# swyoon/Diffusion-by-MaxEntIRL

Hardware: AMD Instinct MI355X
Metric: images/sec (CIFAR-10 DDPM T=10 generation) (higher is better)
Workload: dtype bf16; 1 GPU; CIFAR-10 DDPM U-Net (35.7M params) VARSampler T=10 generation, 256 images/GPU/step, 3x32x32 (BASELINE configs[1]); noise drawn inside the step; global_batch=256, T=10, parallelism=dp1 (independent trajectories, no collective)

## Files before the change

### diffusion-by-maxentirl_amd/csrc/conv1x1_rw.hip

```cpp
#include "conv_common.h"
#include "gn_common.h"

namespace {

#define RW_GPTR(p) ((const __attribute__((address_space(1))) void*)(p))
#define RW_LPTR(p) ((__attribute__((address_space(3))) void*)(p))
#define RW_WAIT_VM(n) asm volatile("s_waitcnt vmcnt(%0)" ::"n"(n) : "memory")
__device__ __forceinline__ void rw_barrier() { asm volatile("s_waitcnt lgkmcnt(0)\n\ts_barrier" ::: "memory"); }

constexpr int RW_CHUNK = 64 * 256;
constexpr int RW_RO = 64 * 256;
constexpr int RW_TBL = 128 * 8;

struct RwGn {
    const float* ab;
    bf16* y;
    int HW, silu;
};

__device__ __forceinline__ void rw_wait_vm(int n) {
    switch (__builtin_amdgcn_readfirstlane(n)) {
#define RW_C(k) case k: RW_WAIT_VM(k); break;
#define RW_C8(k) RW_C(k) RW_C(k + 1) RW_C(k + 2) RW_C(k + 3) RW_C(k + 4) RW_C(k + 5) RW_C(k + 6) RW_C(k + 7)
    RW_C8(0) RW_C8(8) RW_C8(16) RW_C8(24) RW_C8(32) RW_C8(40) RW_C8(48) RW_C8(56)
#undef RW_C8
#undef RW_C
    default: RW_WAIT_VM(0);
    }
}

template <int NCH, int R, bool RES, bool GN>
__global__ __launch_bounds__(256, ((NCH > 3 || R > 4) ? 1 : 2)) void conv1x1_rw_kernel(ConvArgs p, RwGn q) {
    static_assert(R - 1 <= 4 * NCH && R >= 3 && 4 * (R - 2) + 4 * (RES ? 8 : 4) < 64, "ring depth");
    static_assert(!(GN && RES) && (!GN || 5 * (R - 2) + 4 * 4 + 4 * (R - 1) < 64), "GN side output: no residual, vmcnt range");
    constexpr int BOPS = RES ? 8 : 4;
    constexpr int NYOUNG = 4 * (R - 2);
    extern __shared__ __attribute__((aligned(1024))) char smem[];
    char* const ring = smem;

    const int tid = threadIdx.x, lane = tid & 63, h = lane >> 5;
    const int wave = __builtin_amdgcn_readfirstlane(tid >> 6);
    char* const ro = smem + R * RW_CHUNK + wave * 4096;
    char* const tbl = smem + R * RW_CHUNK + RW_RO;
    const int xcd = blockIdx.x & 7, j = blockIdx.x >> 3;
    const int cot = j % p.CT;
    const int nstreams = (gridDim.x >> 3) / p.CT * 8;
    const int stream = (j / p.CT) * 8 + xcd;
    const int ntiles = stream < p.PT ? (p.PT - stream + nstreams - 1) / nstreams : 0;
    if (ntiles == 0) return;

    bf16x8 A[NCH * 8];
// ... 35 lines not shown
                                             RW_LPTR(ring + slot * RW_CHUNK + (wave * 4 + u) * 1024), 16, 0, 0);
    };
    int rpx[4], rc8[4];
#pragma unroll
    for (int i = 0; i < 4; ++i) {
        rpx[i] = i * 16 + (lane >> 2);
        rc8[i] = ((lane & 3) ^ ((rpx[i] >> 1) & 3)) * 8;
    }
    auto tile_off = [&](int tile, int i) -> size_t {
        return ((size_t)(stream + tile * nstreams) * 64 + rpx[i]) * p.Cout + cot * 128 + wave * 32 + rc8[i];
    };
    auto issue_residual = [&](int tile) {
#pragma unroll
        for (int i = 0; i < 4; ++i)
            __builtin_amdgcn_global_load_lds(RW_GPTR(p.residual + tile_off(tile, i)), RW_LPTR(ro + i * 1024), 16, 0, 0);
    };

    const int gtot = ntiles * NCH;
    if (RES) issue_residual(0);
#pragma unroll
    for (int g = 0; g < R - 1; ++g)
        if (g < gtot) issue_chunk(g / NCH, g % NCH, g);

    int boff[8];
    {
        const int px = lane & 31;
#pragma unroll
        for (int ks = 0; ks < 8; ++ks) boff[ks] = px * 256 + (((ks * 2 + h) ^ (px & 15)) << 4);
    }

    const int gnp = GN ? 4 / p.CT : 0;
    const int gs = tid & 15, gpx0 = cot * (64 / p.CT) + (tid >> 4);

    int slot = 0;
    for (int ti = 0; ti < ntiles; ++ti) {
        f32x16 acc[2];
#pragma unroll
        for (int nb = 0; nb < 2; ++nb)
#pragma unroll
            for (int r = 0; r < 16; ++r) acc[nb][r] = 0.f;
#pragma unroll
        for (int c = 0; c < NCH; ++c) {
            const int g = ti * NCH + c;
            const int kmax = R - 1 - c > 0 ? (R - 1 - c + NCH - 1) / NCH : 0;
            const int nbnd = ti < kmax ? ti : kmax;
            if (g + R - 2 >= gtot) RW_WAIT_VM(0);
            else if (GN) rw_wait_vm(5 * (R - 2) + nbnd * BOPS + (g < R - 1 ? g : R - 1) * gnp);
            else if (nbnd == 0) RW_WAIT_VM(NYOUNG);
            else if (nbnd == 1) RW_WAIT_VM(NYOUNG + BOPS);
            else if (nbnd == 2) RW_WAIT_VM(NYOUNG + 2 * BOPS);
            else if (nbnd == 3) RW_WAIT_VM(NYOUNG + 3 * BOPS);
            else RW_WAIT_VM(NYOUNG + 4 * BOPS);
            rw_barrier();
            {
                const int gi = g + R - 1;
                const int si = slot == 0 ? R - 1 : slot - 1;
                if (gi < gtot) issue_chunk(ti + (c + R - 1) / NCH, (c + R - 1) % NCH, si);
            }
            const char* img = ring + slot * RW_CHUNK;
#pragma unroll
            for (int ks = 0; ks < 8; ++ks)
#pragma unroll
                for (int nb = 0; nb < 2; ++nb) {
                    const bf16x8 b = *reinterpret_cast<const bf16x8*>(img + boff[ks] + nb * (32 * 256));
                    acc[nb] = __builtin_amdgcn_mfma_f32_32x32x16_bf16(A[c * 8 + ks], b, acc[nb], 0, 0, 0);
                }
            if constexpr (GN) {
                float ga[8], gb[8];
                const f32x4* t = reinterpret_cast<const f32x4*>(tbl + slot * RW_TBL + gs * 64);
#pragma unroll
                for (int i = 0; i < 4; ++i) {
                    const f32x4 v = t[i];
                    ga[2 * i] = v[0]; gb[2 * i] = v[1]; ga[2 * i + 1] = v[2]; gb[2 * i + 1] = v[3];
                }
                bf16* const yt = q.y + (size_t)(stream + ti * nstreams) * 64 * (NCH * 128) + c * 128 + gs * 8;
                for (int i = 0; i < gnp; ++i) {
                    const int px = gpx0 + 16 * i;
                    const bf16x8 v = *reinterpret_cast<const bf16x8*>(img + px * 256 + ((gs ^ (px & 15)) << 4));
                    *reinterpret_cast<bf16x8*>(yt + (size_t)px * (NCH * 128)) = gn_norm8(v, ga, gb, q.silu);
                }
            }
            slot = slot + 1 == R ? 0 : slot + 1;
        }
        if (RES) {
            if ((ti + 1) * NCH + R - 1 > gtot) RW_WAIT_VM(0);
            else RW_WAIT_VM(4 * NCH);
        }
#pragma unroll
        for (int nb = 0; nb < 2; ++nb) {
            const int px = nb * 32 + (lane & 31);
#pragma unroll
            for (int g4 = 0; g4 < 4; ++g4) {
                char* a = ro + px * 64 + ((g4 ^ ((px >> 1) & 3)) << 4) + 8 * h;
                f32x4 v;
#pragma unroll
                for (int e = 0; e < 4; ++e) v[e] = acc[nb][4 * g4 + e] + bv[g4][e];
                if (RES) {
                    const bf16x4 r = *reinterpret_cast<const bf16x4*>(a);
#pragma unroll
                    for (int e = 0; e < 4; ++e) v[e] += (float)r[e];
                }
                bf16x4 o;
#pragma unroll
                for (int e = 0; e < 4; ++e) o[e] = (bf16)dxmi_act_lin(v[e], slope);
                *reinterpret_cast<bf16x4*>(a) = o;
            }
        }
        asm volatile("s_waitcnt lgkmcnt(0)" ::: "memory");
        {
            bf16x8 v[4];
#pragma unroll
            for (int i = 0; i < 4; ++i) v[i] = *reinterpret_cast<const bf16x8*>(ro + i * 1024 + lane * 16);
#pragma unroll
            for (int i = 0; i < 4; ++i) *reinterpret_cast<bf16x8*>(reinterpret_cast<bf16*>(p.out) + tile_off(ti, i)) = v[i];
        }
        if (RES && ti + 1 < ntiles) issue_residual(ti + 1);
    }
}

template <int NCH, int R>
int rw_launch(const ConvPlan& p, hipStream_t st) {
    static bool attr_set = false;
    if (!attr_set) {
        (void)hipFuncSetAttribute(reinterpret_cast<const void*>(conv1x1_rw_kernel<NCH, R, true, false>), hipFuncAttributeMaxDynamicSharedMemorySize, 160 * 1024);
        (void)hipFuncSetAttribute(reinterpret_cast<const void*>(conv1x1_rw_kernel<NCH, R, false, false>), hipFuncAttributeMaxDynamicSharedMemorySize, 160 * 1024);
        attr_set = true;
    }
    const RwGn none = {};
    if (p.args.residual) hipLaunchKernelGGL((conv1x1_rw_kernel<NCH, R, true, false>), dim3(p.grid), dim3(256), p.lds, st, p.args, none);
    else hipLaunchKernelGGL((conv1x1_rw_kernel<NCH, R, false, false>), dim3(p.grid), dim3(256), p.lds, st, p.args, none);
    DXMI_CHECK_LAUNCH("dxmi_conv2d_fwd(1x1 rw)");
    return DXMI_OK;
}

template <int NCH, int R>
int rw_launch_gn(const ConvArgs& b, const RwGn& g, int grid, hipStream_t st) {
    const size_t lds = (size_t)R * (RW_CHUNK + RW_TBL) + RW_RO;
    static bool attr_set = false;
    if (!attr_set) {
        (void)hipFuncSetAttribute(reinterpret_cast<const void*>(conv1x1_rw_kernel<NCH, R, false, true>), hipFuncAttributeMaxDynamicSharedMemorySize, 160 * 1024);
        attr_set = true;
    }
    hipLaunchKernelGGL((conv1x1_rw_kernel<NCH, R, false, true>), dim3(grid), dim3(256), lds, st, b, g);
    DXMI_CHECK_LAUNCH("dxmi_groupnorm_silu_shortcut");
    return DXMI_OK;
}

int rw_grid(ConvArgs& b) {
    const int K = b.C0 + b.C1;
    b.PT = (int)((long)b.N * b.OH * b.OW / 64);
// ... 11 lines not shown
    const int K = a.C0 + a.C1;
    if (K % 128 != 0 || a.C0 % 128 != 0 || K > 512 || a.Cout % 128 != 0 || a.Cout / 128 > 32) return false;
    const long px = (long)a.N * a.OH * a.OW;
    if (px % 64 != 0 || px / 64 < 512) return false;
    const int nch = K / 128;
    p->kind = ConvKernel::rw; p->t0 = nch; p->t1 = nch > 3 ? 6 : 3;
    p->grid = rw_grid(p->args);
    p->lds = (size_t)p->t1 * RW_CHUNK + RW_RO;
    p->id = 500000 + nch * 1000 + p->t1 * 10 + (a.residual ? 1 : 0);
    return true;
}

int conv1x1_rw_launch(const ConvPlan& p, hipStream_t st) {
    switch (p.t0) {
    case 1: return rw_launch<1, 3>(p, st);
    case 2: return rw_launch<2, 3>(p, st);
    case 3: return rw_launch<3, 3>(p, st);
    default: return rw_launch<4, 6>(p, st);
    }
}

static int gn_shortcut_nch(const dxmi_conv_desc* d, int groups) {
    if (!d || d->ksize != 1 || d->stride != 1 || d->pad != 0 || d->upsample || d->residual || d->addvec || d->mask_src || d->gn_stats ||
        d->gn_out || d->act != DXMI_ACT_NONE || d->variant != 0 || d->in_mode != DXMI_IN_NHWC_BF16 || d->out_mode != DXMI_OUT_NHWC_BF16)
        return 0;
    const int K = d->C0 + d->C1, CT = d->Cout / 128;
    if (d->IH != d->OH || d->IW != d->OW || (d->OH * d->OW) % 64 != 0) return 0;
    if (CT != 1 && CT != 2 && CT != 4) return 0;
    if (groups <= 0 || groups > 32 || K % groups != 0 || (K / groups) % 2 != 0 || d->C1 % 8 != 0) return 0;
    ConvPlan p;
    return conv_plan(d, &p) == DXMI_OK && p.kind == ConvKernel::rw ? p.t0 : 0;
}

extern "C" int dxmi_groupnorm_silu_shortcut_supported(const dxmi_conv_desc* d, int32_t groups) {
    return gn_shortcut_nch(d, groups) > 0 ? 1 : 0;
}

extern "C" int dxmi_groupnorm_silu_shortcut(const dxmi_conv_desc* d, const float* stats0, int32_t P0, const float* stats1, int32_t P1,
                                            const float* gamma, const float* beta, int32_t groups, float eps, int32_t apply_silu, void* y,
                                            float* ab_workspace, void* stream) {
    DXMI_CHECK_ARG(d && d->in0 && d->wpacked && d->out && y && ab_workspace && stats0 && gamma && beta && P0 > 0,
                   "dxmi_groupnorm_silu_shortcut: null pointer");
    DXMI_CHECK_ARG(d->C1 == 0 || (d->in1 && stats1 && P1 > 0), "dxmi_groupnorm_silu_shortcut: C1>0 needs in1 and stats1");
    const int nch = gn_shortcut_nch(d, groups);
    if (nch == 0) return 1;
    const int HW = d->OH * d->OW;
    int rc = gn_finalize_launch(stats0, P0, d->C0, stats1, P1, d->C1, gamma, beta, ab_workspace, d->N, HW, groups, eps, (hipStream_t)stream);
    if (rc != DXMI_OK) return rc;
    ConvArgs b = {};
    b.in0 = (const bf16*)d->in0; b.in1 = (const bf16*)d->in1; b.w = (const bf16*)d->wpacked; b.bias = d->bias; b.out = d->out;
    b.N = d->N; b.IH = d->IH; b.IW = d->IW; b.C0 = d->C0; b.C1 = d->C1; b.OH = d->OH; b.OW = d->OW; b.Cout = d->Cout;
    b.ksize = 1; b.stride = 1; b.act = DXMI_ACT_NONE; b.in_mode = DXMI_IN_NHWC_BF16; b.out_mode = DXMI_OUT_NHWC_BF16;
    b.CB = (d->Cout + 31) / 32;
    const int grid = rw_grid(b);
    const RwGn g = {ab_workspace, (bf16*)y, HW, apply_silu ? 1 : 0};
    const hipStream_t st = (hipStream_t)stream;
    switch (nch) {
    case 1: return rw_launch_gn<1, 3>(b, g, grid, st);
    case 2: return rw_launch_gn<2, 3>(b, g, grid, st);
    case 3: return rw_launch_gn<3, 3>(b, g, grid, st);
    default: return rw_launch_gn<4, 6>(b, g, grid, st);
    }
}
```

### diffusion-by-maxentirl_amd/csrc/conv1x1_rw8.hip

```cpp
#include "conv_common.h"

namespace {

#define R8_GPTR(p) ((const __attribute__((address_space(1))) void*)(p))
#define R8_LPTR(p) ((__attribute__((address_space(3))) void*)(p))
#define R8_WAIT_VM(n) asm volatile("s_waitcnt vmcnt(%0)" ::"n"(n) : "memory")
__device__ __forceinline__ void r8_barrier() { asm volatile("s_waitcnt lgkmcnt(0)\n\ts_barrier" ::: "memory"); }

constexpr int R8_CHUNK = 64 * 256;
constexpr int R8_RMAX = 6;
constexpr int r8_ring(int nk) { return (nk + 1) / 2 + 1 < R8_RMAX ? (nk + 1) / 2 + 1 : R8_RMAX; }
constexpr int r8_lds(int nk) { return r8_ring(nk) * R8_CHUNK + 8 * 4096 + 1024; }

template <int NK, bool RES>
__global__ __launch_bounds__(512, 1) void conv1x1_rw8_kernel(ConvArgs p) {
    constexpr int NCH = (NK + 1) / 2;
    constexpr bool TAIL = (NK & 1) != 0;
    constexpr int R = r8_ring(NK);
    constexpr int BOPS = RES ? 8 : 4;
    constexpr int NYOUNG = 2 * (R - 2);
    static_assert(NCH >= 3 && R - 1 <= NCH && NYOUNG + BOPS < 64, "ring depth: at most one tile boundary inside the ring");
    extern __shared__ __attribute__((aligned(1024))) char smem[];
    char* const ring = smem;
    float* const btab = reinterpret_cast<float*>(smem + R * R8_CHUNK + 8 * 4096);

    const int tid = threadIdx.x, lane = tid & 63, h = lane >> 5;
    const int wave = __builtin_amdgcn_readfirstlane(tid >> 6);
    char* const ro = smem + R * R8_CHUNK + wave * 4096;
    const int xcd = blockIdx.x & 7, j = blockIdx.x >> 3;
    const int cot = j % p.CT;
    const int nstreams = (gridDim.x >> 3) / p.CT * 8;
    const int stream = (j / p.CT) * 8 + xcd;
    const int ntiles = stream < p.PT ? (p.PT - stream + nstreams - 1) / nstreams : 0;
    if (ntiles == 0) return;
    const int co0 = cot * 256 + wave * 32;
    const bool active = co0 < p.Cout;

    if (tid < 256) btab[tid] = (p.bias && cot * 256 + tid < p.Cout) ? p.bias[cot * 256 + tid] : 0.f;
    bf16x8 A[NK * 4];
    {
        const int cb = active ? cot * 8 + wave : p.CB - 1;
        const bf16x8* wf = reinterpret_cast<const bf16x8*>(p.w) + (size_t)cb * 64 + lane;
#pragma unroll
        for (int ks = 0; ks < NK * 4; ++ks) A[ks] = wf[(size_t)ks * p.CB * 64];
    }
    const float slope = dxmi_act_slope(p.act);

    const int dpx0 = wave * 8 + (lane >> 4);
    const int K = NK * 64;
    auto issue_chunk = [&](int tile, int c, int slot) {
        const size_t P0 = (size_t)(stream + tile * nstreams) * 64;
#pragma unroll
        for (int u = 0; u < 2; ++u) {
            const int dpx = dpx0 + 4 * u;
            int ch = c * 128 + (((lane & 15) ^ (dpx & 15)) << 3);
            if (TAIL) ch = ch < K - 8 ? ch : K - 8;
            const bf16* g = ch < p.C0 ? p.in0 + (P0 + dpx) * p.C0 + ch : p.in1 + (P0 + dpx) * p.C1 + (ch - p.C0);
            __builtin_amdgcn_global_load_lds(R8_GPTR(g), R8_LPTR(ring + slot * R8_CHUNK + (wave * 2 + u) * 1024), 16, 0, 0);
        }
    };
    const int rpx0 = lane >> 2, rc8 = ((lane & 3) ^ ((lane >> 3) & 3)) * 8;
    auto tile_off = [&](int tile, int i) -> size_t {
        return ((size_t)(stream + tile * nstreams) * 64 + rpx0 + 16 * i) * p.Cout + co0 + rc8;
    };
    auto issue_residual = [&](int tile) {
#pragma unroll
        for (int i = 0; i < 4; ++i)
            __builtin_amdgcn_global_load_lds(R8_GPTR(p.residual + tile_off(tile, i)), R8_LPTR(ro + i * 1024), 16, 0, 0);
    };

    const int gtot = ntiles * NCH;
    if (RES && active) issue_residual(0);
#pragma unroll
    for (int g = 0; g < R - 1; ++g)
        if (g < gtot) issue_chunk(g / NCH, g % NCH, g);

    const int bpx = lane & 31, bsw = bpx & 15;
    const int brow = bpx * 256;

    int slot = 0;
    for (int ti = 0; ti < ntiles; ++ti) {
        f32x16 acc[2];
#pragma unroll
        for (int nb = 0; nb < 2; ++nb)
#pragma unroll
            for (int r = 0; r < 16; ++r) acc[nb][r] = 0.f;
#pragma unroll
        for (int c = 0; c < NCH; ++c) {
            const int g = ti * NCH + c;
            const bool bnd = active && ti > 0 && c < R - 1;
            if (g + R - 2 >= gtot) R8_WAIT_VM(0);
            else if (!bnd) R8_WAIT_VM(NYOUNG);
            else R8_WAIT_VM(NYOUNG + BOPS);
            r8_barrier();
            {
                const int gi = g + R - 1;
                const int si = slot == 0 ? R - 1 : slot - 1;
                if (gi < gtot) issue_chunk(ti + (c + R - 1) / NCH, (c + R - 1) % NCH, si);
            }
            {
                const char* img = ring + slot * R8_CHUNK + brow;
#pragma unroll
                for (int ks = 0; ks < 8; ++ks) {
                    if (TAIL && c == NCH - 1 && ks >= 4) continue;
                    if (ks == 4) __builtin_amdgcn_sched_barrier(0);
                    const int so = ((ks * 2 + h) ^ bsw) << 4;
#pragma unroll
                    for (int nb = 0; nb < 2; ++nb) {
                        const bf16x8 b = *reinterpret_cast<const bf16x8*>(img + so + nb * (32 * 256));
                        acc[nb] = __builtin_amdgcn_mfma_f32_32x32x16_bf16(A[c * 8 + ks], b, acc[nb], 0, 0, 0);
                    }
                }
            }
            slot = slot + 1 == R ? 0 : slot + 1;
        }
        if (!active) continue;
        if (RES) {
            if ((ti + 1) * NCH + R - 1 > gtot) R8_WAIT_VM(0);
            else R8_WAIT_VM(2 * NCH);
        }
#pragma unroll
        for (int nb = 0; nb < 2; ++nb) {
            const int px = nb * 32 + (lane & 31);
#pragma unroll
            for (int g4 = 0; g4 < 4; ++g4) {
                char* a = ro + px * 64 + ((g4 ^ ((px >> 1) & 3)) << 4) + 8 * h;
                const f32x4 bv = *reinterpret_cast<const f32x4*>(btab + wave * 32 + 8 * g4 + 4 * h);
                f32x4 v;
#pragma unroll
                for (int e = 0; e < 4; ++e) v[e] = acc[nb][4 * g4 + e] + bv[e];
                if (RES) {
                    const bf16x4 r = *reinterpret_cast<const bf16x4*>(a);
#pragma unroll
                    for (int e = 0; e < 4; ++e) v[e] += (float)r[e];
                }
                bf16x4 o;
#pragma unroll
                for (int e = 0; e < 4; ++e) o[e] = (bf16)dxmi_act_lin(v[e], slope);
                *reinterpret_cast<bf16x4*>(a) = o;
            }
        }
        asm volatile("s_waitcnt lgkmcnt(0)" ::: "memory");
        {
            bf16x8 v[4];
#pragma unroll
            for (int i = 0; i < 4; ++i) v[i] = *reinterpret_cast<const bf16x8*>(ro + i * 1024 + lane * 16);
#pragma unroll
            for (int i = 0; i < 4; ++i) *reinterpret_cast<bf16x8*>(reinterpret_cast<bf16*>(p.out) + tile_off(ti, i)) = v[i];
        }
        if (RES && ti + 1 < ntiles) issue_residual(ti + 1);
    }
}

template <int NK>
int r8_launch(const ConvPlan& p, hipStream_t st) {
    static bool attr_set = false;
    if (!attr_set) {
        (void)hipFuncSetAttribute(reinterpret_cast<const void*>(conv1x1_rw8_kernel<NK, true>), hipFuncAttributeMaxDynamicSharedMemorySize, 160 * 1024);
        (void)hipFuncSetAttribute(reinterpret_cast<const void*>(conv1x1_rw8_kernel<NK, false>), hipFuncAttributeMaxDynamicSharedMemorySize, 160 * 1024);
        attr_set = true;
    }
    if (p.args.residual) hipLaunchKernelGGL((conv1x1_rw8_kernel<NK, true>), dim3(p.grid), dim3(512), p.lds, st, p.args);
    else hipLaunchKernelGGL((conv1x1_rw8_kernel<NK, false>), dim3(p.grid), dim3(512), p.lds, st, p.args);
    DXMI_CHECK_LAUNCH("dxmi_conv2d_fwd(1x1 rw8)");
    return DXMI_OK;
}

}

bool conv1x1_rw8_select(const ConvArgs& a, ConvPlan* p) {
    if (a.in_mode != DXMI_IN_NHWC_BF16 || a.out_mode != DXMI_OUT_NHWC_BF16) return false;
    if (a.ksize != 1 || a.stride != 1 || a.pad != 0 || a.ups != 0 || a.mask_src || a.addvec || a.act == DXMI_ACT_SILU) return false;
    const int K = a.C0 + a.C1;
    ConvPlan rw = *p;
    const bool kok = K == 576 || ((K == 384 || K == 512) && (!conv1x1_rw_select(a, &rw) || (K == 512 && a.Cout >= 1024)));
    if (!kok || a.C0 % 8 != 0 || a.C1 % 8 != 0 || a.Cout % 32 != 0) return false;
    const long px = (long)a.N * a.OH * a.OW;
    if (px % 64 != 0) return false;
    const int PT = (int)(px / 64), CT = (a.Cout + 255) / 256;
    if (CT > 32) return false;
    const int grid = 8 * CT * (32 / CT);
    const int nstreams = (grid >> 3) / CT * 8;
    if (PT < 2 * nstreams) return false;
    p->args.PT = PT; p->args.CT = CT; p->args.tile_px = 64;
    p->kind = ConvKernel::rw8; p->t0 = K / 64;
    p->grid = grid;
    p->lds = r8_lds(K / 64);
    p->id = 550000 + (K / 64) * 10 + (a.residual ? 1 : 0);
    return true;
}

int conv1x1_rw8_launch(const ConvPlan& p, hipStream_t st) {
    switch (p.t0) {
    case 6: return r8_launch<6>(p, st);
    case 8: return r8_launch<8>(p, st);
    default: return r8_launch<9>(p, st);
    }
}
```

### diffusion-by-maxentirl_amd/csrc/conv_common.h

```cpp
#pragma once
#include "common.h"

struct ConvArgs {
    const bf16* in0;
    const bf16* in1;
    const bf16* w;
    const float* bias;
    const float* addvec;
    const bf16* residual;
    const bf16* mask_src;
    void* out;
    int N, IH, IW, C0, C1, OH, OW, Cout;
    int ksize, stride, pad, ups, act, addvec_ld, in_mode, out_mode;
    int P, pre_act;
    int TWl, THl, SUBS;
    int HH, HWd;
    int PT, CT, CB, KST;
    int tile_px;
    int lds_buf;
    float mask_slope;
    int stagger;
    int RP, SP;
    float* gn_stats;
    bf16* gn_out;
// ... 129 lines not shown
    }
}

enum class ConvKernel { igemm, pipe, stream1x1, stem, ws, ws8, sm, rw, rw8, head };

struct ConvPlan {
    ConvKernel kind;
    int t0, t1, t2;
    ConvArgs args;
    int grid;
    size_t lds;
    int id;
    int stats_tile;
    bool gn_out;
};

bool conv_ws_select(const ConvArgs& a, ConvPlan* p);
bool conv_ws8_select(const ConvArgs& a, ConvPlan* p);
bool conv_sm_select(const ConvArgs& a, ConvPlan* p);
bool conv1x1_rw_select(const ConvArgs& a, ConvPlan* p);
bool conv1x1_rw8_select(const ConvArgs& a, ConvPlan* p);
bool conv_head_select(const ConvArgs& a, ConvPlan* p);
bool conv_stem_select(const ConvArgs& a, ConvPlan* p);
bool conv_pipe_select(const ConvArgs& a, ConvPlan* p);
int conv_ws_launch(const ConvPlan& p, hipStream_t st);
int conv_ws8_launch(const ConvPlan& p, hipStream_t st);
int conv_sm_launch(const ConvPlan& p, hipStream_t st);
int conv1x1_rw_launch(const ConvPlan& p, hipStream_t st);
int conv1x1_rw8_launch(const ConvPlan& p, hipStream_t st);
int conv_head_launch(const ConvPlan& p, hipStream_t st);
int conv_stem_launch(const ConvPlan& p, hipStream_t st);
int conv_pipe_launch(const ConvPlan& p, hipStream_t st);

template <typename T>
bool conv_zero_page(const void*& page, const T& symbol) {
    void* zp = nullptr;
    if (!page && hipGetSymbolAddress(&zp, symbol) == hipSuccess) page = zp;
    return page != nullptr;
}

int conv_plan(const dxmi_conv_desc* d, ConvPlan* p);
```

### diffusion-by-maxentirl_amd/dxmi_hip/_lib.py

```python
import ctypes
import os

_HERE = os.path.dirname(os.path.abspath(__file__))
LIB_PATH = os.environ.get("DXMI_LIB") or os.path.join(_HERE, "libdxmi_hip.so")

c_void_p, c_int, c_float, c_int64 = ctypes.c_void_p, ctypes.c_int32, ctypes.c_float, ctypes.c_int64


class ConvDesc(ctypes.Structure):

    _fields_ = [
        ("in0", c_void_p), ("in1", c_void_p), ("wpacked", c_void_p), ("bias", c_void_p),
        ("addvec", c_void_p), ("residual", c_void_p), ("out", c_void_p),
        ("N", c_int), ("IH", c_int), ("IW", c_int), ("C0", c_int), ("C1", c_int),
        ("OH", c_int), ("OW", c_int), ("Cout", c_int),
        ("ksize", c_int), ("stride", c_int), ("pad", c_int), ("upsample", c_int), ("act", c_int),
        ("addvec_ld", c_int), ("in_mode", c_int), ("out_mode", c_int), ("variant", c_int),
        ("mask_src", c_void_p), ("mask_slope", c_float), ("gn_stats", c_void_p),
        ("gn_out", c_void_p), ("gn_gamma", c_void_p), ("gn_beta", c_void_p), ("gn_eps", c_float), ("gn_groups", c_int), ("gn_flags", c_int),
    ]


class PackItem(ctypes.Structure):

    _fields_ = [("w", c_void_p), ("dst", c_void_p), ("Cout", c_int), ("Cin", c_int), ("ksize", c_int), ("transpose_flip", c_int),
                ("k27", c_int)]


SIGNATURES = {
    "dxmi_last_error": (ctypes.c_char_p, []),
    "dxmi_version": (c_int, []),
    "dxmi_device_check": (c_int, []),
    "dxmi_set_tuning": (c_int, [ctypes.c_char_p, c_int]),
    "dxmi_get_tuning": (c_int, [ctypes.c_char_p, ctypes.POINTER(c_int)]),
    "dxmi_conv2d_fwd": (c_int, [ctypes.POINTER(ConvDesc), c_void_p]),
    "dxmi_conv2d_kernel_id": (c_int, [ctypes.POINTER(ConvDesc)]),
    "dxmi_conv2d_gn_stats_partials": (c_int, [ctypes.POINTER(ConvDesc)]),
    "dxmi_conv2d_gn_fuse_supported": (c_int, [ctypes.POINTER(ConvDesc)]),
    "dxmi_conv_ws_last_clock": (c_int, [ctypes.POINTER(ctypes.c_uint64)]),
    "dxmi_gn_block_stats_partials": (c_int, [c_int]),
    "dxmi_gn_block_stats": (c_int, [c_void_p, c_void_p, c_int, c_int, c_int, c_void_p]),
    "dxmi_gn_stats_fold": (c_int, [c_void_p, c_void_p, c_int, c_int, c_int, c_int, c_void_p]),
    "dxmi_groupnorm_apply": (c_int, [c_void_p, c_int, c_void_p, c_int, c_void_p, c_int, c_void_p, c_int, c_void_p, c_void_p, c_void_p, c_int,
                                     c_void_p, c_int, c_int, c_int, c_float, c_int, c_void_p]),
    "dxmi_groupnorm_apply_split": (c_int, [c_void_p, c_int, c_void_p, c_int, c_void_p, c_int, c_void_p, c_int, c_void_p, c_void_p, c_void_p, c_int,
                                           c_void_p, c_void_p, c_int, c_int, c_int, c_float, c_int, c_void_p]),
    "dxmi_groupnorm_silu_shortcut_supported": (c_int, [ctypes.POINTER(ConvDesc), c_int]),
    "dxmi_groupnorm_silu_shortcut": (c_int, [ctypes.POINTER(ConvDesc), c_void_p, c_int, c_void_p, c_int, c_void_p, c_void_p, c_int, c_float,
                                             c_int, c_void_p, c_void_p, c_void_p]),
    "dxmi_gn_blockstats_to_generic": (c_int, [c_void_p, c_int, c_int, c_void_p, c_int, c_int, c_void_p, c_int, c_int, c_int, c_void_p]),
    "dxmi_attention_fwd_lse_supported": (c_int, [c_int, c_int, c_int]),
    "dxmi_attention_fwd_lse": (c_int, [c_void_p, c_void_p, c_void_p, c_int, c_int, c_int, c_int, c_float, c_void_p]),
    "dxmi_attention_bwd_lse": (c_int, [c_void_p, c_void_p, c_void_p, c_void_p, c_void_p, c_void_p, c_int, c_int, c_int, c_int, c_float, c_void_p]),
    "dxmi_gn_ss_grads": (c_int, [c_void_p, c_void_p, c_int, c_void_p, c_void_p, c_void_p, c_void_p, c_void_p, c_int, c_int, c_void_p]),
    "dxmi_fid_stats_workspace_bytes": (c_int64, [c_int64, c_int]),
    "dxmi_fid_stats": (c_int, [c_void_p, c_int64, c_int, c_void_p, c_void_p, c_void_p, c_void_p]),
    "dxmi_knn_radii_workspace_bytes": (c_int64, [c_int64, c_int, c_int, c_int]),
    "dxmi_knn_radii": (c_int, [c_void_p, c_int64, c_int, c_int, c_int, c_void_p, c_void_p, c_void_p]),
    "dxmi_pr_membership_workspace_bytes": (c_int64, [c_int64, c_int64]),
    "dxmi_pr_membership": (c_int, [c_void_p, c_int64, c_void_p, c_void_p, c_int64, c_void_p, c_int, c_void_p, c_void_p, c_void_p, c_void_p]),
    "dxmi_inception_score_workspace_bytes": (c_int64, [c_int64, c_int, c_int]),
    "dxmi_inception_score": (c_int, [c_void_p, c_int64, c_int, c_void_p, c_int, c_int, c_void_p, c_void_p, c_void_p]),
    "dxmi_packed_conv_weight_bytes": (c_int64, [c_int, c_int, c_int, c_int]),
    "dxmi_pack_conv_weights": (c_int, [ctypes.POINTER(PackItem), c_int, c_void_p]),
    "dxmi_pack_conv_weight": (c_int, [c_void_p, c_void_p, c_int, c_int, c_int, c_int, c_int, c_void_p]),
    "dxmi_conv2d_wgrad_workspace_bytes": (c_int64, [c_int] * 6),
    "dxmi_conv2d_wgrad_plan": (c_int, [c_int] * 12 + [c_void_p]),
    "dxmi_conv2d_wgrad": (c_int, [c_void_p, c_int, c_void_p, c_int, c_void_p, c_void_p, c_void_p] + [c_int] * 11 + [c_void_p]),
    "dxmi_conv2d_wgrad_bias": (c_int, [c_void_p, c_int, c_void_p, c_int, c_void_p, c_void_p, c_void_p, c_void_p] + [c_int] * 11 + [c_void_p]),
    "dxmi_groupnorm_silu_bwd": (c_int, [c_void_p, c_int, c_void_p, c_int] + [c_void_p] * 9 + [c_int, c_int, c_int, c_float, c_int, c_void_p]),
    "dxmi_bgemm_bf16": (c_int, [c_void_p, c_void_p, c_void_p, c_int, c_int, c_int, c_int64, c_int64, c_int, c_int, c_int64, c_int64, c_int, c_int, c_int64, c_int64, c_int, c_int, c_float, c_int, c_int, c_void_p]),
    "dxmi_softmax_bwd": (c_int, [c_void_p, c_void_p, c_void_p, c_void_p, c_int64, c_int, c_void_p]),
    "dxmi_attention_bwd_supported": (c_int, [c_int, c_int, c_int]),
    "dxmi_attention_bwd_workspace_bytes": (c_int64, [c_int, c_int, c_int]),
    "dxmi_attention_bwd": (c_int, [c_void_p, c_void_p, c_void_p, c_void_p, c_void_p, c_int, c_int, c_int, c_int, c_float, c_void_p]),
    "dxmi_colsum_bf16": (c_int, [c_void_p, c_void_p, c_void_p, c_int64, c_int, c_int, c_void_p]),
    "dxmi_colsum_blocks_bf16": (c_int, [c_void_p, c_void_p, c_int64, c_int, c_int, c_void_p]),
    "dxmi_colsum_f32": (c_int, [c_void_p, c_void_p, c_int, c_int, c_int, c_void_p]),
    "dxmi_pool_act_bwd": (c_int, [c_void_p, c_void_p, c_void_p, c_int, c_int, c_int, c_int, c_int, c_float, c_void_p]),
    "dxmi_value_head_bwd": (c_int, [c_void_p, c_void_p, c_void_p, c_void_p, c_void_p, c_int, c_int, c_int, c_void_p]),
# ... 112 lines not shown
```

### diffusion-by-maxentirl_amd/dxmi_hip/ops.py

```python
import ctypes
import os

import torch

from . import _lib
from . import graph as _graph
from ._lib import ConvDesc, check, load

ACT_NONE, ACT_LEAKY02, ACT_RELU, ACT_SILU = 0, 1, 2, 3
IN_NHWC_BF16, IN_NCHW_F32_K27 = 0, 1
OUT_NHWC_BF16, OUT_NCHW_F32 = 0, 1


_RAW_STREAM = getattr(torch._C, "_cuda_getCurrentRawStream", None)
_GET_DEVICE = getattr(torch._C, "_cuda_getDevice", None)


def _stream():
    if _RAW_STREAM is not None and _GET_DEVICE is not None:
        return ctypes.c_void_p(_RAW_STREAM(_GET_DEVICE()))
    return ctypes.c_void_p(torch.cuda.current_stream().cuda_stream)


def _tree_fingerprint(module):
# ... 686 lines not shown
    if (C // groups) % 2 != 0 or C0 % 8 != 0 or C1 % 8 != 0:
        return None
    assert x.dtype == torch.bfloat16 and x.is_contiguous() and C == pw.Cin
    assert in1 is None or (in1.dtype == torch.bfloat16 and in1.is_contiguous() and in1.shape[:3] == x.shape[:3])
    assert gamma.dtype == torch.float32 and beta.dtype == torch.float32 and gamma.numel() == C and beta.numel() == C
    st0, st1 = stats[0], (stats[1] if in1 is not None else None)
    assert tuple(st0.buf.shape) == (N, st0.P, C0 // 2, 2) and (st1 is None or tuple(st1.buf.shape) == (N, st1.P, C1 // 2, 2))
    Cout = pw.Cout
    sc = torch.empty((N, H, W, Cout), dtype=torch.bfloat16, device=x.device)
    d = ConvDesc()
    d.in0, d.in1, d.wpacked = x.data_ptr(), (in1.data_ptr() if in1 is not None else None), pw.buf.data_ptr()
    d.bias = bias.data_ptr() if bias is not None else None
    d.out = sc.data_ptr()
    d.N, d.IH, d.IW, d.C0, d.C1, d.OH, d.OW, d.Cout = N, H, W, C0, C1, H, W, Cout
    d.ksize, d.stride, d.pad, d.upsample, d.act = 1, 1, 0, 0, ACT_NONE
    d.in_mode, d.out_mode = IN_NHWC_BF16, OUT_NHWC_BF16
    lib = load()
    key = ("gn_shortcut", N, H, W, C0, C1, Cout, groups, bias is not None)
    ok = _STATS_P.get(key)
    if ok is None:
        ok = _STATS_P[key] = int(lib.dxmi_groupnorm_silu_shortcut_supported(ctypes.byref(d), groups))
    if not ok:
        return None
    y = torch.empty((N, H, W, C), dtype=torch.bfloat16, device=x.device)
    ab = torch.empty((N, C, 2), dtype=torch.float32, device=x.device)
    px = N * H * W
    _prof("groupnorm", "gn_shortcut", 2.0 * px * C * Cout, 2.0 * (2 * px * C + px * Cout + C * Cout), lambda: check(
        lib.dxmi_groupnorm_silu_shortcut(ctypes.byref(d), _ptr(st0.buf), st0.P, _ptr(st1.buf) if st1 is not None else None,
                                         st1.P if st1 is not None else 0, _ptr(gamma), _ptr(beta), groups, float(eps), int(silu),
                                         _ptr(y), _ptr(ab), _stream()), "dxmi_groupnorm_silu_shortcut"))
    return y, sc


def gn_blockstats_to_generic(st0, st1, N, HW, C0, C1, groups=32):
    lib = load()
    ws = torch.empty(lib.dxmi_groupnorm_generic_workspace_bytes(N, HW, C0 + C1) // 4, dtype=torch.float32, device=st0.buf.device)
    check(lib.dxmi_gn_blockstats_to_generic(_ptr(st0.buf), st0.P, C0, _ptr(st1.buf) if st1 is not None else None, st1.P if st1 is not None else 0,
                                            C1, _ptr(ws), N, HW, groups, _stream()), "dxmi_gn_blockstats_to_generic")
    return ws


def groupnorm_generic(x, gamma, beta, *, in1=None, groups=32, eps=1e-5, silu=True, out=None, scale_shift=None, saved=None):
    _need_cuda(x, in1, gamma, beta, out, scale_shift)
    N, H, W, C0 = x.shape
    C1 = in1.shape[3] if in1 is not None else 0
    C = C0 + C1
    assert x.dtype == torch.bfloat16 and x.is_contiguous()
    if out is None:
        out = torch.empty((N, H, W, C), dtype=torch.bfloat16, device=x.device)
    ss_ld = 0
    if scale_shift is not None:
        assert scale_shift.dtype == torch.float32 and scale_shift.stride(-1) == 1 and scale_shift.shape[1] == 2 * C
        ss_ld = scale_shift.stride(0)
    lib = load()
    nbytes = lib.dxmi_groupnorm_generic_workspace_bytes(N, H * W, C)
    if saved is not None:
        ws = torch.empty(nbytes // 4, dtype=torch.float32, device=x.device)
        saved.append(ws)
    else:
        ws = _workspace(nbytes, x.device)
    _prof("groupnorm", "generic", 0.0, 4.0 * N * H * W * C, lambda: check(
        lib.dxmi_groupnorm_generic_fwd(_ptr(x), C0, _ptr(in1), C1, _ptr(gamma), _ptr(beta), _ptr(scale_shift), ss_ld, _ptr(out),
                                       _ptr(ws), N, H * W, groups, float(eps), int(silu), _stream()), "dxmi_groupnorm_generic_fwd"))
    return out


# ... 966 lines not shown
```

### include/dxmi_hip.h

```cpp
#ifndef DXMI_HIP_H
#define DXMI_HIP_H

#include <stdint.h>

#ifdef __cplusplus
extern "C" {
#endif

#define DXMI_OK            0
#define DXMI_EINVAL       -1
#define DXMI_ELAUNCH      -2
#define DXMI_ENODEV       -3

#define DXMI_ACT_NONE      0
#define DXMI_ACT_LEAKY02   1
#define DXMI_ACT_RELU      2
#define DXMI_ACT_SILU      3

#define DXMI_IN_NHWC_BF16     0
#define DXMI_IN_NCHW_F32_K27  1
#define DXMI_IN_ROWS_F32      2
#define DXMI_OUT_NHWC_BF16    0
#define DXMI_OUT_NCHW_F32     1
#define DXMI_OUT_ROWS_F32     2
// ... 98 lines not shown
int64_t dxmi_attention_bwd_workspace_bytes(int32_t N, int32_t T, int32_t heads);
int dxmi_attention_bwd(const void* qkv, const void* o, const void* dout, void* dqkv, void* workspace, int32_t N, int32_t T,
                       int32_t C, int32_t heads, float scale, void* stream);

int dxmi_attention_fwd_lse_supported(int32_t T, int32_t C, int32_t heads);
int dxmi_attention_fwd_lse(const void* qkv, void* out, float* lse, int32_t N, int32_t T, int32_t C, int32_t heads, float scale, void* stream);
int dxmi_attention_bwd_lse(const void* qkv, const void* o, const void* dout, void* dqkv, const float* lse_fwd, void* workspace, int32_t N,
                           int32_t T, int32_t C, int32_t heads, float scale, void* stream);

int dxmi_pool_act_bwd(const void* dout, const void* act_out, void* din, int32_t N, int32_t H, int32_t W,
                      int32_t C, int32_t pool, float slope, void* stream);
int dxmi_value_head_bwd(const void* feat, const float* w, const float* dy, void* dfeat, float* s,
                        int32_t N, int32_t HW, int32_t C, void* stream);

int dxmi_groupnorm_silu_fwd(const void* in0, int32_t C0, const void* in1, int32_t C1,
                            const float* gamma, const float* beta, void* out,
                            int32_t N, int32_t HW, int32_t groups, float eps,
                            int32_t apply_silu, void* stream);

int dxmi_gn_block_stats_partials(int32_t HW);
int dxmi_gn_block_stats(const void* x, float* stats, int32_t N, int32_t HW, int32_t C, void* stream);
int dxmi_gn_stats_fold(const float* stats, float* out, int32_t N, int32_t P, int32_t C, int32_t group, void* stream);
int dxmi_groupnorm_apply(const void* in0, int32_t C0, const float* stats0, int32_t P0, const void* in1, int32_t C1,
                         const float* stats1, int32_t P1, const float* gamma, const float* beta, const float* scale_shift,
                         int32_t ss_ld, void* out, int32_t N, int32_t HW, int32_t groups, float eps, int32_t apply_silu,
                         void* stream);

int dxmi_groupnorm_apply_split(const void* in0, int32_t C0, const float* stats0, int32_t P0, const void* in1, int32_t C1,
                               const float* stats1, int32_t P1, const float* gamma, const float* beta,
                               const float* scale_shift, int32_t ss_ld, void* out, float* ab_workspace, int32_t N, int32_t HW,
                               int32_t groups, float eps, int32_t apply_silu, void* stream);

int dxmi_groupnorm_silu_shortcut_supported(const dxmi_conv_desc* d, int32_t groups);
int dxmi_groupnorm_silu_shortcut(const dxmi_conv_desc* d, const float* stats0, int32_t P0, const float* stats1, int32_t P1,
                                 const float* gamma, const float* beta, int32_t groups, float eps, int32_t apply_silu, void* y,
                                 float* ab_workspace, void* stream);

int dxmi_gn_blockstats_to_generic(const float* stats0, int32_t P0, int32_t C0, const float* stats1, int32_t P1, int32_t C1,
                                  float* generic_stats, int32_t N, int32_t HW, int32_t groups, void* stream);

int dxmi_gn_ss_grads(const float* g, const float* scale_shift, int32_t ss_ld, const float* gamma, const float* beta,
                     float* d_scale_shift, float* dgamma, float* dbeta, int32_t N, int32_t C, void* stream);

int dxmi_attention_fwd(const void* qkv, void* out, int32_t N, int32_t T, int32_t C,
                       int32_t heads, float scale, void* stream);

int dxmi_attention_proj_supported(int32_t T, int32_t C, int32_t heads);
int dxmi_pack_attn_proj_weight(const float* w_oi, void* dst, void* stream);
int dxmi_attention_proj_fwd(const void* qkv, const void* wproj_packed, const float* bias, const void* residual, void* out,
                            float* gn_stats, int32_t N, int32_t T, int32_t C, int32_t heads, float scale, void* stream);

int dxmi_attn_block_supported(int32_t T, int32_t C, int32_t heads, int32_t groups);
int64_t dxmi_attn_block_packed_bytes(void);
int dxmi_attn_block_pack(const float* wq, const float* bq, const float* wk, const float* wv, const float* bv,
                         const float* wproj, const float* bproj, float scale, void* dst, void* stream);
int dxmi_attn_block_fwd(const void* x, const float* stats, int32_t P, const float* gamma, const float* beta, float eps,
                        const void* packed, void* out, float* out_stats, int32_t N, int32_t T, int32_t C, void* stream);

int dxmi_timestep_embedding(const float* t, float* out, int32_t N, int32_t dim, int32_t order,
                            float max_period, void* stream);
int dxmi_linear_fwd(const float* x, const void* wpacked, const float* bias, float* out,
                    int32_t P, int32_t K, int32_t M, int32_t pre_act, int32_t post_act,
                    void* stream);
int dxmi_linear_splitk_slices(int32_t P, int32_t K, int32_t M);
int dxmi_linear_splitk(const float* x, const void* wpacked, float* partials, int32_t P, int32_t K, int32_t M, int32_t pre_act,
                       void* stream);
// ... 287 lines not shown
```

Before: 7295 images/s.

## Route GroupNorm-SiLU shortcut conv through 8-wave rw8 kernel with fused GN side output

Adds a GN side-output mode to the 512-thread rw8 1x1 conv kernel. One wave DMAs the per-channel GN affine table into LDS, and every wave normalises its staged input pixels and writes y while the conv runs. The groupnorm_silu_shortcut path selects this kernel for K=512, Cout=256 shapes with enough pixel tiles, and falls back to the 4-wave rw kernel otherwise. It also adds optional timestamp instrumentation and a kernel-id query, at the cost of more complex vmcnt accounting in the new path.

Result: no change. 7358 images/s, median of 6 (+0.9%).

```diff
diff --git a/diffusion-by-maxentirl_amd/csrc/conv1x1_rw.hip b/diffusion-by-maxentirl_amd/csrc/conv1x1_rw.hip
--- a/diffusion-by-maxentirl_amd/csrc/conv1x1_rw.hip
+++ b/diffusion-by-maxentirl_amd/csrc/conv1x1_rw.hip
@@ -1,5 +1,13 @@
 #include "conv_common.h"
 #include "gn_common.h"
+
+#ifdef DXMI_RW_STAMPS
+__device__ unsigned g_rw_stamps[16][4][8];
+extern "C" int dxmi_debug_read_rw_stamps(void* dst, int bytes) {
+    return (int)hipMemcpyFromSymbol(dst, HIP_SYMBOL(g_rw_stamps), bytes, 0, hipMemcpyDeviceToHost);
+}
+#define RW_STAMP(v) do { __builtin_amdgcn_sched_barrier(0); v = (unsigned)__builtin_amdgcn_s_memtime(); __builtin_amdgcn_sched_barrier(0); } while (0)
+#endif
 
 namespace {
 
@@ -11,12 +19,6 @@
 constexpr int RW_CHUNK = 64 * 256;
 constexpr int RW_RO = 64 * 256;
 constexpr int RW_TBL = 128 * 8;
-
-struct RwGn {
-    const float* ab;
-    bf16* y;
-    int HW, silu;
-};
 
 __device__ __forceinline__ void rw_wait_vm(int n) {
     switch (__builtin_amdgcn_readfirstlane(n)) {
@@ -118,6 +120,10 @@
     const int gnp = GN ? 4 / p.CT : 0;
     const int gs = tid & 15, gpx0 = cot * (64 / p.CT) + (tid >> 4);
 
+#ifdef DXMI_RW_STAMPS
+    unsigned sacc[6] = {0, 0, 0, 0, 0, 0}, st0, st1, st1b, st2, st3, st4 = 0, stfirst;
+    RW_STAMP(stfirst);
+#endif
     int slot = 0;
     for (int ti = 0; ti < ntiles; ++ti) {
         f32x16 acc[2];
@@ -130,6 +136,9 @@
             const int g = ti * NCH + c;
             const int kmax = R - 1 - c > 0 ? (R - 1 - c + NCH - 1) / NCH : 0;
             const int nbnd = ti < kmax ? ti : kmax;
+#ifdef DXMI_RW_STAMPS
+            RW_STAMP(st0);
+#endif
             if (g + R - 2 >= gtot) RW_WAIT_VM(0);
             else if (GN) rw_wait_vm(5 * (R - 2) + nbnd * BOPS + (g < R - 1 ? g : R - 1) * gnp);
             else if (nbnd == 0) RW_WAIT_VM(NYOUNG);
@@ -138,11 +147,17 @@
             else if (nbnd == 3) RW_WAIT_VM(NYOUNG + 3 * BOPS);
             else RW_WAIT_VM(NYOUNG + 4 * BOPS);
             rw_barrier();
+#ifdef DXMI_RW_STAMPS
+            RW_STAMP(st1);
+#endif
             {
                 const int gi = g + R - 1;
                 const int si = slot == 0 ? R - 1 : slot - 1;
                 if (gi < gtot) issue_chunk(ti + (c + R - 1) / NCH, (c + R - 1) % NCH, si);
             }
+#ifdef DXMI_RW_STAMPS
+            RW_STAMP(st1b);
+#endif
             const char* img = ring + slot * RW_CHUNK;
 #pragma unroll
             for (int ks = 0; ks < 8; ++ks)
@@ -151,6 +166,9 @@
                     const bf16x8 b = *reinterpret_cast<const bf16x8*>(img + boff[ks] + nb * (32 * 256));
                     acc[nb] = __builtin_amdgcn_mfma_f32_32x32x16_bf16(A[c * 8 + ks], b, acc[nb], 0, 0, 0);
                 }
+#ifdef DXMI_RW_STAMPS
+            RW_STAMP(st2);
+#endif
             if constexpr (GN) {
                 float ga[8], gb[8];
                 const f32x4* t = reinterpret_cast<const f32x4*>(tbl + slot * RW_TBL + gs * 64);
@@ -160,12 +178,28 @@
                     ga[2 * i] = v[0]; gb[2 * i] = v[1]; ga[2 * i + 1] = v[2]; gb[2 * i + 1] = v[3];
                 }
                 bf16* const yt = q.y + (size_t)(stream + ti * nstreams) * 64 * (NCH * 128) + c * 128 + gs * 8;
+#ifdef DXMI_RW_STAMPS
+                st4 = st2;
+#endif
                 for (int i = 0; i < gnp; ++i) {
                     const int px = gpx0 + 16 * i;
                     const bf16x8 v = *reinterpret_cast<const bf16x8*>(img + px * 256 + ((gs ^ (px & 15)) << 4));
+#ifdef DXMI_RW_STAMPS
+                    const bf16x8 o = gn_norm8(v, ga, gb, q.silu);
+                    RW_STAMP(st3);
+                    sacc[3] += st3 - st4;
+                    *reinterpret_cast<bf16x8*>(yt + (size_t)px * (NCH * 128)) = o;
+                    RW_STAMP(st4);
+                    sacc[4] += st4 - st3;
+#else
                     *reinterpret_cast<bf16x8*>(yt + (size_t)px * (NCH * 128)) = gn_norm8(v, ga, gb, q.silu);
+#endif
                 }
             }
+#ifdef DXMI_RW_STAMPS
+            if (!GN) st4 = st2;
+            sacc[0] += st1 - st0; sacc[1] += st1b - st1; sacc[2] += st2 - st1b;
+#endif
             slot = slot + 1 == R ? 0 : slot + 1;
         }
         if (RES) {
@@ -201,7 +235,20 @@
             for (int i = 0; i < 4; ++i) *reinterpret_cast<bf16x8*>(reinterpret_cast<bf16*>(p.out) + tile_off(ti, i)) = v[i];
         }
         if (RES && ti + 1 < ntiles) issue_residual(ti + 1);
-    }
+#ifdef DXMI_RW_STAMPS
+        RW_STAMP(st0);
+        sacc[5] += st0 - st4;
+#endif
+    }
+#ifdef DXMI_RW_STAMPS
+    if (GN && blockIdx.x < 16 && lane < 8) {
+        const unsigned v[8] = {sacc[0], sacc[1], sacc[2], sacc[3], sacc[4], sacc[5], (unsigned)gtot, st0 - stfirst};
+        unsigned o = v[0];
+#pragma unroll
+        for (int i = 1; i < 8; ++i) o = lane == i ? v[i] : o;
+        g_rw_stamps[blockIdx.x][wave][lane] = o;
+    }
+#endif
 }
 
 template <int NCH, int R>
@@ -279,8 +326,30 @@
     return conv_plan(d, &p) == DXMI_OK && p.kind == ConvKernel::rw ? p.t0 : 0;
 }
 
+static bool gn_shortcut_rw8(const dxmi_conv_desc* d, ConvArgs* b, ConvPlan* p8) {
+    *b = {};
+    b->in0 = (const bf16*)d->in0; b->in1 = (const bf16*)d->in1; b->w = (const bf16*)d->wpacked; b->bias = d->bias; b->out = d->out;
+    b->N = d->N; b->IH = d->IH; b->IW = d->IW; b->C0 = d->C0; b->C1 = d->C1; b->OH = d->OH; b->OW = d->OW; b->Cout = d->Cout;
+    b->ksize = 1; b->stride = 1; b->act = DXMI_ACT_NONE; b->in_mode = DXMI_IN_NHWC_BF16; b->out_mode = DXMI_OUT_NHWC_BF16;
+    b->CB = (d->Cout + 31) / 32;
+#ifdef DXMI_RW_STAMPS
+    return false;
+#else
+    return conv1x1_rw8_gn_select(*b, p8);
+#endif
+}
+
 extern "C" int dxmi_groupnorm_silu_shortcut_supported(const dxmi_conv_desc* d, int32_t groups) {
     return gn_shortcut_nch(d, groups) > 0 ? 1 : 0;
+}
+
+extern "C" int dxmi_groupnorm_silu_shortcut_kernel_id(const dxmi_conv_desc* d, int32_t groups) {
+    const int nch = gn_shortcut_nch(d, groups);
+    if (nch == 0) return 0;
+    ConvArgs b;
+    ConvPlan p8;
+    if (gn_shortcut_rw8(d, &b, &p8)) return p8.id;
+    return 500000 + nch * 1000 + (nch > 3 ? 6 : 3) * 10 + 2;
 }
 
 extern "C" int dxmi_groupnorm_silu_shortcut(const dxmi_conv_desc* d, const float* stats0, int32_t P0, const float* stats1, int32_t P1,
@@ -294,14 +363,12 @@
     const int HW = d->OH * d->OW;
     int rc = gn_finalize_launch(stats0, P0, d->C0, stats1, P1, d->C1, gamma, beta, ab_workspace, d->N, HW, groups, eps, (hipStream_t)stream);
     if (rc != DXMI_OK) return rc;
-    ConvArgs b = {};
-    b.in0 = (const bf16*)d->in0; b.in1 = (const bf16*)d->in1; b.w = (const bf16*)d->wpacked; b.bias = d->bias; b.out = d->out;
-    b.N = d->N; b.IH = d->IH; b.IW = d->IW; b.C0 = d->C0; b.C1 = d->C1; b.OH = d->OH; b.OW = d->OW; b.Cout = d->Cout;
-    b.ksize = 1; b.stride = 1; b.act = DXMI_ACT_NONE; b.in_mode = DXMI_IN_NHWC_BF16; b.out_mode = DXMI_OUT_NHWC_BF16;
-    b.CB = (d->Cout + 31) / 32;
-    const int grid = rw_grid(b);
+    ConvArgs b;
+    ConvPlan p8;
     const RwGn g = {ab_workspace, (bf16*)y, HW, apply_silu ? 1 : 0};
     const hipStream_t st = (hipStream_t)stream;
+    if (gn_shortcut_rw8(d, &b, &p8)) return conv1x1_rw8_gn_launch(p8, g, st);
+    const int grid = rw_grid(b);
     switch (nch) {
     case 1: return rw_launch_gn<1, 3>(b, g, grid, st);
     case 2: return rw_launch_gn<2, 3>(b, g, grid, st);
diff --git a/diffusion-by-maxentirl_amd/csrc/conv1x1_rw8.hip b/diffusion-by-maxentirl_amd/csrc/conv1x1_rw8.hip
--- a/diffusion-by-maxentirl_amd/csrc/conv1x1_rw8.hip
+++ b/diffusion-by-maxentirl_amd/csrc/conv1x1_rw8.hip
@@ -1,4 +1,5 @@
 #include "conv_common.h"
+#include "gn_common.h"
 
 namespace {
 
@@ -11,18 +12,34 @@
 constexpr int R8_RMAX = 6;
 constexpr int r8_ring(int nk) { return (nk + 1) / 2 + 1 < R8_RMAX ? (nk + 1) / 2 + 1 : R8_RMAX; }
 constexpr int r8_lds(int nk) { return r8_ring(nk) * R8_CHUNK + 8 * 4096 + 1024; }
-
-template <int NK, bool RES>
-__global__ __launch_bounds__(512, 1) void conv1x1_rw8_kernel(ConvArgs p) {
+constexpr int R8_TBL = 128 * 8;
+constexpr int R8_TW = 7;
+
+__device__ __forceinline__ void r8_wait_vm(int n) {
+    switch (__builtin_amdgcn_readfirstlane(n)) {
+#define R8_C(k) case k: R8_WAIT_VM(k); break;
+#define R8_C8(k) R8_C(k) R8_C(k + 1) R8_C(k + 2) R8_C(k + 3) R8_C(k + 4) R8_C(k + 5) R8_C(k + 6) R8_C(k + 7)
+    R8_C8(0) R8_C8(8) R8_C8(16) R8_C8(24)
+#undef R8_C8
+#undef R8_C
+    default: R8_WAIT_VM(0);
+    }
+}
+
+template <int NK, bool RES, bool GN>
+__global__ __launch_bounds__(512, 1) void conv1x1_rw8_kernel(ConvArgs p, RwGn q) {
     constexpr int NCH = (NK + 1) / 2;
     constexpr bool TAIL = (NK & 1) != 0;
     constexpr int R = r8_ring(NK);
     constexpr int BOPS = RES ? 8 : 4;
     constexpr int NYOUNG = 2 * (R - 2);
+    constexpr int NYST = 2;
     static_assert(NCH >= 3 && R - 1 <= NCH && NYOUNG + BOPS < 64, "ring depth: at most one tile boundary inside the ring");
+    static_assert(!(GN && (RES || TAIL)) && (!GN || 3 * (R - 2) + NYST * (R - 1) + BOPS < 32), "GN side output: no residual, vmcnt range");
     extern __shared__ __attribute__((aligned(1024))) char smem[];
     char* const ring = smem;
     float* const btab = reinterpret_cast<float*>(smem + R * R8_CHUNK + 8 * 4096);
+    char* const tbl = smem + R * R8_CHUNK + 8 * 4096 + 1024;
 
     const int tid = threadIdx.x, lane = tid & 63, h = lane >> 5;
     const int wave = __builtin_amdgcn_readfirstlane(tid >> 6);
@@ -50,6 +67,12 @@
     const int K = NK * 64;
     auto issue_chunk = [&](int tile, int c, int slot) {
         const size_t P0 = (size_t)(stream + tile * nstreams) * 64;
+        if constexpr (GN) {
+            if (wave == R8_TW) {
+                const int n = (int)P0 / q.HW;
+                __builtin_amdgcn_global_load_lds(R8_GPTR(q.ab + ((size_t)n * K + c * 128) * 2 + lane * 4), R8_LPTR(tbl + slot * R8_TBL), 16, 0, 0);
+            }
+        }
 #pragma unroll
         for (int u = 0; u < 2; ++u) {
             const int dpx = dpx0 + 4 * u;
@@ -78,6 +101,9 @@
     const int bpx = lane & 31, bsw = bpx & 15;
     const int brow = bpx * 256;
 
+    const int gs = lane & 15, gpx0 = wave * 8 + (lane >> 4);
+    const int ndma = 2 + (wave == R8_TW ? 1 : 0);
+
     int slot = 0;
     for (int ti = 0; ti < ntiles; ++ti) {
         f32x16 acc[2];
@@ -89,7 +115,10 @@
         for (int c = 0; c < NCH; ++c) {
             const int g = ti * NCH + c;
             const bool bnd = active && ti > 0 && c < R - 1;
-            if (g + R - 2 >= gtot) R8_WAIT_VM(0);
+            if constexpr (GN) {
+                const int young = gtot - 1 - g < R - 2 ? gtot - 1 - g : R - 2;
+                r8_wait_vm(young * ndma + NYST * (g < R - 1 ? g : R - 1) + (bnd ? BOPS : 0));
+            } else if (g + R - 2 >= gtot) R8_WAIT_VM(0);
             else if (!bnd) R8_WAIT_VM(NYOUNG);
             else R8_WAIT_VM(NYOUNG + BOPS);
             r8_barrier();
@@ -112,6 +141,23 @@
                     }
                 }
             }
+            if constexpr (GN) {
+                float ga[8], gb[8];
+                const f32x4* t = reinterpret_cast<const f32x4*>(tbl + slot * R8_TBL + gs * 64);
+#pragma unroll
+                for (int i = 0; i < 4; ++i) {
+                    const f32x4 v = t[i];
+                    ga[2 * i] = v[0]; gb[2 * i] = v[1]; ga[2 * i + 1] = v[2]; gb[2 * i + 1] = v[3];
+                }
+                const char* img = ring + slot * R8_CHUNK;
+                bf16* const yt = q.y + ((size_t)(stream + ti * nstreams) * 64 + gpx0) * K + c * 128 + gs * 8;
+#pragma unroll
+                for (int u = 0; u < NYST; ++u) {
+                    const int px = gpx0 + 4 * u;
+                    const bf16x8 v = *reinterpret_cast<const bf16x8*>(img + px * 256 + ((gs ^ (px & 15)) << 4));
+                    *reinterpret_cast<bf16x8*>(yt + (size_t)(4 * u) * K) = gn_norm8(v, ga, gb, q.silu);
+                }
+            }
             slot = slot + 1 == R ? 0 : slot + 1;
         }
         if (!active) continue;
@@ -156,13 +202,26 @@
 int r8_launch(const ConvPlan& p, hipStream_t st) {
     static bool attr_set = false;
     if (!attr_set) {
-        (void)hipFuncSetAttribute(reinterpret_cast<const void*>(conv1x1_rw8_kernel<NK, true>), hipFuncAttributeMaxDynamicSharedMemorySize, 160 * 1024);
-        (void)hipFuncSetAttribute(reinterpret_cast<const void*>(conv1x1_rw8_kernel<NK, false>), hipFuncAttributeMaxDynamicSharedMemorySize, 160 * 1024);
+        (void)hipFuncSetAttribute(reinterpret_cast<const void*>(conv1x1_rw8_kernel<NK, true, false>), hipFuncAttributeMaxDynamicSharedMemorySize, 160 * 1024);
+        (void)hipFuncSetAttribute(reinterpret_cast<const void*>(conv1x1_rw8_kernel<NK, false, false>), hipFuncAttributeMaxDynamicSharedMemorySize, 160 * 1024);
         attr_set = true;
     }
-    if (p.args.residual) hipLaunchKernelGGL((conv1x1_rw8_kernel<NK, true>), dim3(p.grid), dim3(512), p.lds, st, p.args);
-    else hipLaunchKernelGGL((conv1x1_rw8_kernel<NK, false>), dim3(p.grid), dim3(512), p.lds, st, p.args);
+    const RwGn none = {};
+    if (p.args.residual) hipLaunchKernelGGL((conv1x1_rw8_kernel<NK, true, false>), dim3(p.grid), dim3(512), p.lds, st, p.args, none);
+    else hipLaunchKernelGGL((conv1x1_rw8_kernel<NK, false, false>), dim3(p.grid), dim3(512), p.lds, st, p.args, none);
     DXMI_CHECK_LAUNCH("dxmi_conv2d_fwd(1x1 rw8)");
+    return DXMI_OK;
+}
+
+template <int NK>
+int r8_launch_gn(const ConvPlan& p, const RwGn& g, hipStream_t st) {
+    static bool attr_set = false;
+    if (!attr_set) {
+        (void)hipFuncSetAttribute(reinterpret_cast<const void*>(conv1x1_rw8_kernel<NK, false, true>), hipFuncAttributeMaxDynamicSharedMemorySize, 160 * 1024);
+        attr_set = true;
+    }
+    hipLaunchKernelGGL((conv1x1_rw8_kernel<NK, false, true>), dim3(p.grid), dim3(512), p.lds, st, p.args, g);
+    DXMI_CHECK_LAUNCH("dxmi_groupnorm_silu_shortcut(rw8)");
     return DXMI_OK;
 }
 
@@ -197,3 +256,26 @@
     default: return r8_launch<9>(p, st);
     }
 }
+
+#ifndef R8_GN_K384
+#define R8_GN_K384 0
+#endif
+bool conv1x1_rw8_gn_select(const ConvArgs& a, ConvPlan* p) {
+    const int K = a.C0 + a.C1;
+    if (!(K == 512 || (R8_GN_K384 && K == 384)) || a.Cout != 256 || a.C0 % 8 != 0 || a.C1 % 8 != 0 || a.residual) return false;
+    const long px = (long)a.N * a.OH * a.OW;
+    if (px % 64 != 0 || (a.OH * a.OW) % 64 != 0) return false;
+    const int PT = (int)(px / 64), grid = 256, nstreams = 256;
+    if (PT < 2 * nstreams) return false;
+    p->args = a;
+    p->args.PT = PT; p->args.CT = 1; p->args.tile_px = 64;
+    p->kind = ConvKernel::rw8; p->t0 = K / 64;
+    p->grid = grid;
+    p->lds = r8_lds(K / 64) + r8_ring(K / 64) * R8_TBL;
+    p->id = 550000 + (K / 64) * 10 + 2;
+    return true;
+}
+
+int conv1x1_rw8_gn_launch(const ConvPlan& p, const RwGn& g, hipStream_t st) {
+    return p.t0 == 6 ? r8_launch_gn<6>(p, g, st) : r8_launch_gn<8>(p, g, st);
+}
diff --git a/diffusion-by-maxentirl_amd/csrc/conv_common.h b/diffusion-by-maxentirl_amd/csrc/conv_common.h
--- a/diffusion-by-maxentirl_amd/csrc/conv_common.h
+++ b/diffusion-by-maxentirl_amd/csrc/conv_common.h
@@ -185,6 +185,14 @@
 int conv_stem_launch(const ConvPlan& p, hipStream_t st);
 int conv_pipe_launch(const ConvPlan& p, hipStream_t st);
 
+struct RwGn {
+    const float* ab;
+    bf16* y;
+    int HW, silu;
+};
+bool conv1x1_rw8_gn_select(const ConvArgs& a, ConvPlan* p);
+int conv1x1_rw8_gn_launch(const ConvPlan& p, const RwGn& g, hipStream_t st);
+
 template <typename T>
 bool conv_zero_page(const void*& page, const T& symbol) {
     void* zp = nullptr;
diff --git a/diffusion-by-maxentirl_amd/dxmi_hip/_lib.py b/diffusion-by-maxentirl_amd/dxmi_hip/_lib.py
--- a/diffusion-by-maxentirl_amd/dxmi_hip/_lib.py
+++ b/diffusion-by-maxentirl_amd/dxmi_hip/_lib.py
@@ -46,6 +46,7 @@
     "dxmi_groupnorm_apply_split": (c_int, [c_void_p, c_int, c_void_p, c_int, c_void_p, c_int, c_void_p, c_int, c_void_p, c_void_p, c_void_p, c_int,
                                            c_void_p, c_void_p, c_int, c_int, c_int, c_float, c_int, c_void_p]),
     "dxmi_groupnorm_silu_shortcut_supported": (c_int, [ctypes.POINTER(ConvDesc), c_int]),
+    "dxmi_groupnorm_silu_shortcut_kernel_id": (c_int, [ctypes.POINTER(ConvDesc), c_int]),
     "dxmi_groupnorm_silu_shortcut": (c_int, [ctypes.POINTER(ConvDesc), c_void_p, c_int, c_void_p, c_int, c_void_p, c_void_p, c_int, c_float,
                                              c_int, c_void_p, c_void_p, c_void_p]),
     "dxmi_gn_blockstats_to_generic": (c_int, [c_void_p, c_int, c_int, c_void_p, c_int, c_int, c_void_p, c_int, c_int, c_int, c_void_p]),
diff --git a/diffusion-by-maxentirl_amd/dxmi_hip/ops.py b/diffusion-by-maxentirl_amd/dxmi_hip/ops.py
--- a/diffusion-by-maxentirl_amd/dxmi_hip/ops.py
+++ b/diffusion-by-maxentirl_amd/dxmi_hip/ops.py
@@ -742,6 +742,15 @@
     return y, sc
 
 
+def groupnorm_silu_shortcut_kernel_id(N, H, W, C0, C1, Cout, groups=32):
+    d = ConvDesc()
+    d.in0, d.in1, d.wpacked, d.out = 16, (16 if C1 else None), 16, 16
+    d.N, d.IH, d.IW, d.C0, d.C1, d.OH, d.OW, d.Cout = N, H, W, C0, C1, H, W, Cout
+    d.ksize, d.stride, d.pad, d.upsample, d.act = 1, 1, 0, 0, ACT_NONE
+    d.in_mode, d.out_mode = IN_NHWC_BF16, OUT_NHWC_BF16
+    return int(load().dxmi_groupnorm_silu_shortcut_kernel_id(ctypes.byref(d), groups))
+
+
 def gn_blockstats_to_generic(st0, st1, N, HW, C0, C1, groups=32):
     lib = load()
     ws = torch.empty(lib.dxmi_groupnorm_generic_workspace_bytes(N, HW, C0 + C1) // 4, dtype=torch.float32, device=st0.buf.device)
diff --git a/include/dxmi_hip.h b/include/dxmi_hip.h
--- a/include/dxmi_hip.h
+++ b/include/dxmi_hip.h
@@ -154,6 +154,7 @@
                                int32_t groups, float eps, int32_t apply_silu, void* stream);
 
 int dxmi_groupnorm_silu_shortcut_supported(const dxmi_conv_desc* d, int32_t groups);
+int dxmi_groupnorm_silu_shortcut_kernel_id(const dxmi_conv_desc* d, int32_t groups);
 int dxmi_groupnorm_silu_shortcut(const dxmi_conv_desc* d, const float* stats0, int32_t P0, const float* stats1, int32_t P1,
                                  const float* gamma, const float* beta, int32_t groups, float eps, int32_t apply_silu, void* y,
                                  float* ab_workspace, void* stream);
```
